# SoraKurihara/FFM

Hardware: AMD Instinct MI355X
Metric: agent-steps/sec (whole node), 12×12 grid × 64k envs, 1/2/4/8 GPU (higher is better)
Workload: dtype f32; 1 GPU; ffm_core step, 12x12 room, 32 agents/env, 65536 envs/GPU, neumann, Philox seed 42, on-device auto-reset, steady state (envs desynchronised by a 1000-step untimed burn-in after reset); burn_in_steps=1000, map=12x12, agents_per_env=32, envs_per_gpu=65536, global_envs=65536, parallelism=env-sharded x1

## Files before the change

ffm_amd/csrc/core_group.hip:

```cpp
#include <hip/hip_runtime.h>
#include <stdint.h>

#include <algorithm>
#include <cstdlib>
#include <cstring>

#include "core_common.h"
#include "kernels.h"
#include "lane_common.h"
#include "episode_log.h"
#include "wave_reset.h"

namespace ffm {

namespace {

constexpr int kGroupMaxIters = 16;
constexpr int kGroupPendWords = 8 * kGroupMaxIters / 32;

struct GroupCarve {
    size_t grid, tile, words, posst, kp, keys, pend, dummy, per_wave;
};

template <int G>
__host__ __device__ inline GroupCarve group_carve(int PHW, int TS, int F) {
    GroupCarve c;
    size_t o = 0;
    c.grid = o;  o += a16((size_t)G * PHW * 2);
    c.tile = o;  o += a16((size_t)G * TS * 4);
    c.keys = 0;
    const size_t keys_end = a16((size_t)(F > 0 ? F : 1) * 8);
    if (o < keys_end) o = keys_end;
    c.words = o; o += (size_t)G * 32 * 4;
    c.posst = o;
    c.kp = o;    o += a16((size_t)(((G * 32 + 63) / 64) * 64 + 1) * 2);
    c.pend = o;  o += kGroupPendWords * 4;
    c.dummy = o; o += 4;
    c.per_wave = a16(o);
    return c;
}

__host__ __device__ inline size_t group_shared_bytes(int PHW, int F) {
    return a16((size_t)PHW) + a16((size_t)PHW * 4) + a16((size_t)(F > 0 ? F : 1) * 2) + a16((size_t)PHW * 2);
}

constexpr int kGeomWords = 12;
constexpr int kGeomTableBytes = 64 * kGeomWords * 4;

template <int H, int W, int G>
void group_lane_geom(int lane, int32_t (&w)[kGeomWords]) {
    constexpr int HW = H * W, TS = lane_tile_floats(H, W), Q4 = HW / 4, Q = G * Q4;
    constexpr int NS = (Q + 63) / 64, NSF = Q / 64, HQ = (4 + W) / 4;
    static_assert(NS <= 3 && (4 + W) % 4 == 0 && TS % 4 == 0 && G * 2 * HQ <= 64 && G * TS / 4 <= 255,
                  "geometry table entry");
    uint32_t yfl = 0, senv = 0, tail = 0;
    int lo[3] = {0, 0, 0}, ro[3] = {0, 0, 0}, tlo = 0, tro = 0;
    for (int k = 0; k < 3; k++) w[k] = -1;
    for (int k = 0; k < NS; k++) {
        const int q = k * 64 + lane;
        const int s = q / Q4, c = 4 * (q - s * Q4), y = c % W;
        w[k] = q < Q ? s * TS + 4 + W + c : -1;
        yfl |= (q < Q && y == 0 ? 1u : 0u) << (2 * k);
        yfl |= (q < Q && y == W - 4 ? 2u : 0u) << (2 * k);
        senv |= (uint32_t)(q < Q ? s : 15) << (4 * k);
        lo[k] = q < Q && y != 0 ? w[k] - 1 : 0;
        ro[k] = q < Q && y != W - 4 ? w[k] + 4 : 0;
    }
    if (Q % 64 != 0 && (Q % 64) * 4 == 64) {
        const int q = 4 * 64 * NSF + lane;
        const int s = q / HW, c = q - s * HW, y = c % W, off = s * TS + 4 + W + c;
        tail = (y == 0 ? 1u : 0u) | (y == W - 1 ? 2u : 0u);
        tlo = y != 0 ? off - 1 : 0;
        tro = y != W - 1 ? off + 1 : 0;
    }
    const int s = lane / (2 * HQ), j = lane % (2 * HQ);
    const uint32_t halo = lane < G * 2 * HQ ? (uint32_t)(s * (TS / 4) + (j < HQ ? j : TS / 4 - 2 * HQ + j)) : 255u;
    w[3] = (int32_t)(yfl | (senv << 8) | (tail << 20) | (halo << 24));
    w[4] = lo[0]; w[5] = ro[0]; w[6] = lo[1]; w[7] = ro[1];
    w[8] = tlo; w[9] = tro; w[10] = lo[2]; w[11] = ro[2];
}

__device__ __forceinline__ int cs_pp(uint32_t v) { return (int)(v & 0xFFFFu); }
__device__ __forceinline__ int cs_al(uint32_t v) { return (int)((v >> 16) & 31u); }
__device__ __forceinline__ int cs_s(uint32_t v) { return (int)((v >> 21) & 7u); }
__device__ __forceinline__ bool cs_live(uint32_t v) { return ((v >> 24) & 1u) != 0u; }
__device__ __forceinline__ int cs_xp1(uint32_t v) { return (int)(v >> 25); }

}

#ifndef FFM_GROUP_PROBE_VALU
#define FFM_GROUP_PROBE_VALU 0
#endif
#ifndef FFM_GROUP_PROBE_SALU
#define FFM_GROUP_PROBE_SALU 0
#endif
#ifndef FFM_GROUP_PROBE_DUP
#define FFM_GROUP_PROBE_DUP 0
#endif

#ifndef FFM_GROUP_ABLATE
#define FFM_GROUP_ABLATE 0
#endif

#ifndef FFM_GROUP_TAIL
#define FFM_GROUP_TAIL 1
#endif

#ifndef FFM_GROUP_LADDER
#define FFM_GROUP_LADDER 4
#endif

#ifndef FFM_GROUP_PF
#define FFM_GROUP_PF 0
#endif

#ifndef FFM_GROUP_STAGGER
#define FFM_GROUP_STAGGER 0
#endif

#ifndef FFM_GROUP_WAVES
#define FFM_GROUP_WAVES 6
#endif

#ifndef FFM_GROUP_G
#define FFM_GROUP_G 4
#endif
constexpr int kGroupG = FFM_GROUP_G;
#ifndef FFM_GROUP_G_SMALL
#define FFM_GROUP_G_SMALL 2
#endif
constexpr int kGroupGSmall = FFM_GROUP_G_SMALL;

template <int NB, int HT, int WT, int G, bool KD1, bool EPL>
__global__ __launch_bounds__(256) __attribute__((amdgpu_waves_per_eu(FFM_GROUP_WAVES, 8)))
void core_group_kernel(CoreStepArgs a) {
    extern __shared__ __attribute__((aligned(16))) unsigned char smem[];
    constexpr int H = HT, W = WT, HW = H * W, PW = W + 2, PHW = (H + 2) * PW;
    constexpr int TS = lane_tile_floats(H, W);
    constexpr int Q4 = HW / 4;
    constexpr int Q = G * Q4;
    constexpr int NS = (Q + 63) / 64;
    constexpr int NSF = Q / 64;
    constexpr bool SCALAR_TAIL = NB == 4 && FFM_GROUP_TAIL && Q % 64 != 0 && (Q % 64) * 4 == 64;
    constexpr int MAXC = (G * 32 + 63) / 64;
    constexpr int PWORDS = G * 16;
    static_assert(G >= 1 && G <= 8 && HW % 4 == 0 && H + 1 < 128, "group geometry");
    static_assert(MAXC * 64 >= G * 32 && PWORDS * 4 <= (MAXC * 64 + 1) * 2, "kp spans the chunks; posst fits in it");
    const int A = a.A;
    const int lane = (int)(threadIdx.x & 63);
    const int wv = __builtin_amdgcn_readfirstlane((int)(threadIdx.x >> 6));

    const GroupCarve cv = group_carve<G>(PHW, TS, a.F);
    const float* psff = reinterpret_cast<const float*>(smem + a16((size_t)PHW));
    const uint16_t* pfree = reinterpret_cast<const uint16_t*>(smem + a16((size_t)PHW) + a16((size_t)PHW * 4));
    unsigned char* wbase = smem + group_shared_bytes(PHW, a.F) + (size_t)wv * cv.per_wave;
    uint16_t* const grid = reinterpret_cast<uint16_t*>(wbase + cv.grid);
    float* const tile = reinterpret_cast<float*>(wbase + cv.tile);
    uint32_t* const words = reinterpret_cast<uint32_t*>(wbase + cv.words);
    uint32_t* const posst32 = reinterpret_cast<uint32_t*>(wbase + cv.posst);
    const uint16_t* const posst = reinterpret_cast<const uint16_t*>(wbase + cv.posst);
    uint16_t* const kp = reinterpret_cast<uint16_t*>(wbase + cv.kp);
    unsigned long long* keys = reinterpret_cast<unsigned long long*>(wbase + cv.keys);
    uint32_t* const pend = reinterpret_cast<uint32_t*>(wbase + cv.pend);
    const int kDummy16 = (int)((cv.dummy - cv.grid) / 2);
    const int kDummy32 = (int)((cv.dummy - cv.words) / 4);

    static_assert(G == kGroupG || G == kGroupGSmall, "a geometry table per built group size");
    const int sq4 = a.stage_q4;
    const __amdgpu_buffer_rsrc_t rS = pair_rsrc(a.stage, sq4 * 16 + 2 * kGeomTableBytes);
    const int gtab = sq4 * 16 + (G == kGroupG ? kGeomTableBytes : 0);
    auto geom = [&](int j) {
        return __builtin_bit_cast(uint4, __builtin_amdgcn_raw_buffer_load_b128(rS, lane * 16 + j * 1024, gtab, 0));
    };
    const uint4 gw = geom(0);
    static_assert(NS <= 3, "geometry table entry");
    int toff[NS];
#pragma unroll
    for (int k = 0; k < NS; k++) toff[k] = (int)(k == 0 ? gw.x : k == 1 ? gw.y : gw.z);
    const uint32_t geo = gw.w;
    int lo[NS], ro[NS];
#pragma unroll
    for (int k = 0; k < NS; k++) lo[k] = ro[k] = 0;
    if (NB == 4) {
        const uint4 gb = geom(1);
        lo[0] = (int)gb.x; ro[0] = (int)gb.y;
        if (NS > 1) { lo[1] = (int)gb.z; ro[1] = (int)gb.w; }
        if (NS > 2 && !SCALAR_TAIL) {
            const uint4 gc = geom(2);
            lo[2] = (int)gc.z; ro[2] = (int)gc.w;
        }
    }

    const long long E = a.E;
    const uint32_t ebase = (uint32_t)a.env_base;
    const int Epad = (int)((E + 7) & ~7LL);
    const __amdgpu_buffer_rsrc_t rC = pair_rsrc(a.cnt, Epad * 4);
    const __amdgpu_buffer_rsrc_t rP = pair_rsrc(a.pos, Epad * A * 2 + 4);
    const __amdgpu_buffer_rsrc_t rD = pair_rsrc(a.dff, Epad * HW * 4);
    const int ngroups = (int)((E + G - 1) / G);
    const int wstride = (int)gridDim.x * 4;
    int g = (int)blockIdx.x * 4 + wv;

    struct GState {
        float4 d[NS];
        uint32_t p0, p1;
        int c;
    };
    const __amdgpu_buffer_rsrc_t rZ = pair_rsrc(a.dff, 0);
    auto load = [&](int gg, GState& st) {
        const bool ok = gg >= 0;
        const int e0 = ok ? gg * G : 0;
        const __amdgpu_buffer_rsrc_t rc = ok ? rC : rZ, rp = ok ? rP : rZ, rd = ok ? rD : rZ;
        st.c = (int)__builtin_amdgcn_raw_buffer_load_b32(rc, lane < G ? lane * 4 : kOOB, e0 * 4, 0);
        st.p0 = __builtin_amdgcn_raw_buffer_load_b32(rp, lane < PWORDS ? lane * 4 : kOOB, e0 * A * 2, 0);
        st.p1 = PWORDS > 64 ? __builtin_amdgcn_raw_buffer_load_b32(rp, 64 + lane < PWORDS ? 256 + lane * 4 : kOOB,
                                                                 e0 * A * 2, 0)
                            : 0u;
#pragma unroll
        for (int k = 0; k < NS; k++) {
            const int q = k * 64 + lane;
            st.d[k] = __builtin_bit_cast(float4,
                                         __builtin_amdgcn_raw_buffer_load_b128(rd, q < Q ? q * 16 : kOOB, e0 * HW * 4, 0));
        }
    };
    constexpr int LAD = FFM_GROUP_LADDER;
    constexpr int PF = FFM_GROUP_PF;
    if (FFM_GROUP_STAGGER > 0) {
        const int mine = g < ngroups ? (ngroups - 1 - g) / wstride + 1 : 0;
        const int most = (ngroups - 1) / wstride + 1;
        if (mine < most) __builtin_amdgcn_s_sleep(FFM_GROUP_STAGGER);
    }
    GState cur;
    load(g < ngroups ? g : -1, cur);

    if (LAD >= 1) {
    if ((int)threadIdx.x < sq4)
        reinterpret_cast<uint4*>(smem)[threadIdx.x] = __builtin_bit_cast(
            uint4, __builtin_amdgcn_raw_buffer_load_b128(rS, (int)threadIdx.x * 16, 0, 0));
    static_assert((PHW * 2) % 8 == 0 && PHW * 2 / 8 <= 64, "8-B grid copies, one per lane");
    if (lane < PHW * 2 / 8) {
        const int pm16 = (int)(a16((size_t)PHW) + a16((size_t)PHW * 4) + a16((size_t)(a.F > 0 ? a.F : 1) * 2));
        const auto mw = __builtin_amdgcn_raw_buffer_load_b64(rS, lane * 8, pm16, 0);
#pragma unroll
        for (int s = 0; s < G; s++)
            *reinterpret_cast<uint2*>(reinterpret_cast<unsigned char*>(grid) + s * (PHW * 2) + lane * 8) =
                __builtin_bit_cast(uint2, mw);
    }
    if ((geo >> 24) != 255u) reinterpret_cast<float4*>(tile)[geo >> 24] = make_float4(0.f, 0.f, 0.f, 0.f);
    if (lane < kGroupPendWords) pend[lane] = 0u;
    __syncthreads();
    }

    unsigned c_steps = 0, c_exits = 0, c_resets = 0;
    constexpr uint32_t mW = (uint32_t)(((1ull << 32) + (unsigned)W - 1) / (unsigned)W);
    const int g_first = g;
    for (int iter = 0; g < ngroups; g += wstride, iter++) {
        const int e0 = g * G;
        const int nenv = (int)min((long long)G, E - e0);
        if (LAD <= 2) {
            const __amdgpu_buffer_rsrc_t rq = pair_rsrc(a.pos + e0 * A, (nenv * A * 2 + 3) & ~3);
            __builtin_amdgcn_raw_buffer_store_b32(cur.p0, rq, lane < PWORDS ? lane * 4 : kOOB, 0, 0);
            if (PWORDS > 64)
                __builtin_amdgcn_raw_buffer_store_b32(cur.p1, rq, 64 + lane < PWORDS ? 256 + lane * 4 : kOOB, 0, 0);
            __builtin_amdgcn_raw_buffer_store_b32((unsigned)cur.c, pair_rsrc(a.cnt + e0, nenv * 4),
                                                  lane < G ? lane * 4 : kOOB, 0, 0);
            c_steps += (unsigned)A * (unsigned)nenv;
        }
        if (LAD <= 1) {
            const __amdgpu_buffer_rsrc_t rq = pair_rsrc(a.dff + e0 * HW, nenv * HW * 4);
#pragma unroll
            for (int k = 0; k < NS; k++) {
                const int q = k * 64 + lane;
                buf_st4(rq, q < Q ? q * 16 : kOOB, cur.d[k]);
            }
            GState nx;
            load(g + wstride < ngroups ? g + wstride : -1, nx);
            cur = nx;
            continue;
        }

        GState nxt;
        const int gn = g + wstride < ngroups ? g + wstride : -1;
#pragma unroll
        for (int k = 0; k < NS; k++)
            if (k < NSF || toff[k] >= 0) *reinterpret_cast<float4*>(tile + toff[k]) = cur.d[k];
        if (PF == 3) load(gn, nxt);
        unsigned long long rsm = 0ull;
        if (LAD == 2) wave_sync();
        if (LAD >= 3) {
        if (lane < PWORDS) posst32[lane] = cur.p0;
        if (PWORDS > 64 && 64 + lane < PWORDS) posst32[64 + lane] = cur.p1;
        int S[G + 1];
        S[0] = 0;
#pragma unroll
        for (int s = 0; s < G; s++) S[s + 1] = S[s] + __builtin_amdgcn_readlane(cur.c, s);
        const int T = S[G];
        c_steps += (unsigned)T;
        wave_sync();

        uint32_t cs[MAXC], cr[MAXC];
#pragma unroll
        for (int c = 0; c < MAXC; c++) {
            cs[c] = (uint32_t)(PW + 1) | (1u << 25);
            cr[c] = 15u;
            if (c * 64 < T) {
                const int j = c * 64 + lane;
                int s = 0, st = 0;
#pragma unroll
                for (int q = 1; q < G; q++) {
                    const bool ge = j >= S[q];
                    s += ge ? 1 : 0;
                    st = ge ? S[q] : st;
                }
                const bool live = j < T;
                const int al = live ? j - st : 0;
                const uint32_t p = posst[live ? s * A + al : 0];
                const int x = (int)__umulhi(p, mW);
                const int y = (int)p - x * W;
                const int pp = live ? (x + 1) * PW + y + 1 : PW + 1;
                grid[live ? s * PHW + pp : kDummy16] = (uint16_t)(DirCodes::kAgent | (uint32_t)al | (DirCodes::kNoDir << 8));
                cs[c] = (uint32_t)pp | ((uint32_t)al << 16) | ((uint32_t)s << 21) | ((live ? 1u : 0u) << 24) |
                        ((uint32_t)(live ? x + 1 : 1) << 25);
            }
        }
        wave_sync();

        if (PF == 2) load(gn, nxt);
#pragma unroll
        for (int c = 0; c < MAXC; c++) {
            if (LAD == 3) cr[c] = DirCodes::kNoDir;
            if (LAD >= 4 && c * 64 < T) {
                const uint32_t v = cs[c];
                const int pp = cs_pp(v), al = cs_al(v), s = cs_s(v);
                const bool live = cs_live(v);
                const uint32_t genv = ebase + (uint32_t)e0 + (uint32_t)s;
                const uint4 pb = philox(make_uint4(a.t, genv, (uint32_t)al, kPurDecide << 28), a.key0, a.key1);
                words[live ? s * 32 + al : kDummy32] = pb.w;
                const uint16_t* gk = grid + s * PHW;
                const float* dk = tile + s * TS;
                const int dd0 = 3 - 2 * cs_xp1(v);
                bool to_exit = false;
                uint32_t slot = lane_decide<NB, true, KD1>(pp, PW, gk, psff, dk, dd0, a.kS32, a.kD32, pb.x, to_exit);
                slot = live ? slot : kNoReq;
                if (slot == kPending)
                    slot = NB == 4 ? lane_decide_exact<NB, true>(pp, PW, gk, psff, dk, dd0, a.kS32, a.kD32,
                                                                 u53(pb.x, pb.y))
                                   : lane_decide_exact_arr<NB, true>(pp, PW, gk, psff, dk, dd0, a.kS32, a.kD32,
                                                               u53(pb.x, pb.y));
                const uint32_t sd = slot <= (uint32_t)NB ? slot : DirCodes::kNoDir;
                grid[live ? s * PHW + pp : kDummy16] =
                    (uint16_t)(DirCodes::kAgent | (uint32_t)al | (sd << 8) | ((pb.z >> 31) << 12));
                cr[c] = sd | ((to_exit ? 1u : 0u) << 4);
#if FFM_GROUP_PROBE_DUP
                if (c == MAXC - 1) {
                    uint32_t salt;
                    asm volatile("v_mov_b32 %0, 0" : "=v"(salt));
                    const uint4 pb2 = philox(make_uint4(a.t, genv, (uint32_t)al + salt, kPurDecide << 28), a.key0,
                                             a.key1);
                    bool te2 = false;
                    const uint32_t slot2 =
                        lane_decide<NB, true, KD1>(pp, PW, gk, psff, dk, dd0, a.kS32, a.kD32, pb2.x, te2);
                    asm volatile("" ::"v"(slot2), "v"(pb2.w), "v"(te2 ? 1u : 0u));
                }
#endif
            }
        }
        wave_sync();

        if (PF == 1) load(gn, nxt);
        unsigned long long km[MAXC];
        int kept = 0;
#pragma unroll
        for (int c = 0; c < MAXC; c++) {
            km[c] = 0ull;
            if (c * 64 < T) {
                const uint32_t v = cs[c];
                const int pp = cs_pp(v), al = cs_al(v), s = cs_s(v);
                const bool live = cs_live(v);
                const uint32_t sd = cr[c] & 15u;
                const bool to_exit = (cr[c] & 16u) != 0u;
                const uint32_t slot = sd == DirCodes::kNoDir ? (uint32_t)kNoReq : sd;
                const uint16_t* gk = grid + s * PHW;
                const int r = (int)slot_cell_k<NB, PW>(slot, pp);
                const bool req = slot <= (uint32_t)NB;
                const bool moving = req && r != pp;
                bool granted = req && !moving;
                if (LAD >= 4) {
                    const int rt = moving ? r : pp;
                    int m = 0, k = 0, o = 0x7F;
                    uint32_t zo = 0u;
#pragma unroll
                    for (int d = 0; d < NB; d++) {
                        const uint32_t cc = gk[rt - nb_dx<NB>(d) * PW - nb_dy<NB>(d)];
                        const bool is = (cc & DirCodes::kAgent) != 0u && ((cc >> 8) & 0xFu) == (uint32_t)d;
                        const int who = (int)(cc & DirCodes::kIdx);
                        m += is ? 1 : 0;
                        k += (is && who < al) ? 1 : 0;
                        const bool lower = is && who < o;
                        zo = lower ? (cc >> 12) & 1u : zo;
                        o = lower ? who : o;
                    }
                    granted = moving ? m == 1 : granted;
                    if (moving && m > 1) {
                        const uint32_t w = words[s * 32 + o];
                        const uint32_t genv = ebase + (uint32_t)e0 + (uint32_t)s;
                        const int kk = philox_friction(zo << 31, w, (uint32_t)m, a.key0, a.key1, a.t, genv,
                                                       (uint32_t)o);
                        granted = kk == k;
                    }
                }
                if (granted)
                    __hip_atomic_fetch_add(tile + s * TS + pp + 3 - 2 * cs_xp1(v), 1.0f, __ATOMIC_RELAXED,
                                           __HIP_MEMORY_SCOPE_WAVEFRONT);
                const int np = granted ? r : pp;
                const bool keep = live && !(granted && to_exit);
                km[c] = __ballot(keep);
                const int kpv = kept + lanes_below(km[c]);
                kept += __popcll(km[c]);
                cr[c] = (uint32_t)np | ((keep ? 1u : 0u) << 16) | ((uint32_t)kpv << 17);
            }
        }

#pragma unroll
        for (int c = 0; c < MAXC; c++) {
            if (c * 64 < T) {
                const uint32_t v = cs[c];
                kp[c * 64 + lane] = (uint16_t)(cr[c] >> 17);
                grid[cs_live(v) ? cs_s(v) * PHW + cs_pp(v) : kDummy16] = 0;
            }
        }
        if (lane == 0) kp[T] = (uint16_t)kept;
        c_exits += (unsigned)(T - kept);
        wave_sync();
#pragma unroll
        for (int c = 0; c < MAXC; c++) {
            if (c * 64 < T) {
                const uint32_t v = cs[c], w = cr[c];
                const int j = c * 64 + lane;
                const int s = cs_s(v);
                const bool keep = ((w >> 16) & 1u) != 0u;
                const int start = j - cs_al(v);
                const int newidx = (int)(w >> 17) - (int)kp[cs_live(v) ? start : 0];
                __builtin_amdgcn_raw_buffer_store_b16((uint16_t)unpad((int)(w & 0xFFFFu), PW), rP,
                                                      keep ? (s * A + newidx) * 2 : kOOB, e0 * A * 2, 0);
            }
        }
        int Sl = T, Sh = T;
#pragma unroll
        for (int s = 0; s < G; s++) {
            Sl = lane == s ? S[s] : Sl;
            Sh = lane == s ? S[s + 1] : Sh;
        }
        const int nk = (int)kp[Sh] - (int)kp[Sl];
        const bool rs = a.auto_reset && lane < nenv && nk == 0;
        rsm = __ballot(rs);
        __builtin_amdgcn_raw_buffer_store_b32((unsigned)(rs ? a.N : nk), rC, lane < G ? lane * 4 : kOOB, e0 * 4, 0);
        if (rsm) {
            c_resets += (unsigned)__popcll(rsm);
            if (a.episodes && rs) a.episodes[e0 + lane] += 1;
            if (lane == 0) pend[iter >> 2] |= (uint32_t)rsm << (8 * (iter & 3));
        }
        if (EPL && (rsm || !a.auto_reset))
            eplog_end_wave(a, lane < nenv && nk == 0 && Sh > Sl, rs, e0 + lane, a.t, lane);
        }

        if (PF == 0 || LAD < 3) load(gn, nxt);

#if FFM_GROUP_PROBE_VALU > 0 || FFM_GROUP_PROBE_SALU > 0
        {
            uint32_t pv = (uint32_t)lane, ps = (uint32_t)g;
#pragma unroll
            for (int i = 0; i < FFM_GROUP_PROBE_VALU; i++) asm volatile("v_add_u32 %0, %0, 1" : "+v"(pv));
#pragma unroll
            for (int i = 0; i < FFM_GROUP_PROBE_SALU; i++) asm volatile("s_add_u32 %0, %0, 1" : "+s"(ps));
            asm volatile("" ::"v"(pv), "s"(ps));
        }
#endif
        if (SCALAR_TAIL) {
            const int q = 4 * 64 * NSF + lane;
            constexpr int ts = 4 * 64 * NSF / HW, tc = 4 * 64 * NSF - ts * HW;
            static_assert(!SCALAR_TAIL || (4 * 64 * NSF + 63) / HW == ts, "the scalar tail spans envs");
            const float* p = tile + (ts * TS + 4 + W + tc) + lane;
            const float m0 = p[0], mu = p[-W], md = p[W], pl = p[-1], pr = p[1];
            const float ml = (geo & (1u << 20)) ? 0.0f : pl, mr = (geo & (2u << 20)) ? 0.0f : pr;
            const float b0 = a.c0 * m0, bu = a.c0 * mu, bd = a.c0 * md, bl = a.c0 * ml, br = a.c0 * mr;
            float acc = b0;
            acc = acc + a.c1 * bu;
            acc = acc + a.c1 * bd;
            acc = acc + a.c1 * bl;
            acc = acc + a.c1 * br;
            float o = acc < 1e-4f ? 0.0f : acc;
            if (rsm && ((rsm >> ts) & 1ull)) o = 0.0f;
            __builtin_amdgcn_raw_buffer_store_b32(__builtin_bit_cast(uint32_t, o), rD, q * 4, e0 * HW * 4, 0);
        }
#pragma unroll
        for (int k = 0; k < (SCALAR_TAIL ? NSF : NS); k++) {
            const int tb = toff[k];
            if (k >= NSF && tb < 0) continue;
            const bool yl = ((geo >> (2 * k)) & 1u) != 0u, yr = ((geo >> (2 * k)) & 2u) != 0u;
            const float* p = tile + tb;
            float b[3][6];
#pragma unroll
            for (int dx = -1; dx <= 1; dx++) {
                const float4 u = *reinterpret_cast<const float4*>(p + dx * W);
                b[dx + 1][1] = a.c0 * u.x; b[dx + 1][2] = a.c0 * u.y;
                b[dx + 1][3] = a.c0 * u.z; b[dx + 1][4] = a.c0 * u.w;
                if (NB == 4 && dx != 0) continue;
                b[dx + 1][0] = a.c0 * tile[NB == 4 ? lo[k] : yl ? 0 : tb + dx * W - 1];
                b[dx + 1][5] = a.c0 * tile[NB == 4 ? ro[k] : yr ? 0 : tb + dx * W + 4];
            }
            float o[4];
#pragma unroll
            for (int jj = 0; jj < 4; jj++) {
                float acc = b[1][jj + 1];
#pragma unroll
                for (int d = 0; d < NB; d++) {
                    const float t = a.c1 * b[1 + nb_dx<NB>(d)][jj + 1 + nb_dy<NB>(d)];
                    acc = acc + t;
                }
                o[jj] = acc < 1e-4f ? 0.0f : acc;
            }
            float4 out = make_float4(o[0], o[1], o[2], o[3]);
            if (rsm) {
                if ((rsm >> ((geo >> (8 + 4 * k)) & 15u)) & 1ull) out = make_float4(0.f, 0.f, 0.f, 0.f);
            }
            __builtin_amdgcn_raw_buffer_store_b128(__builtin_bit_cast(__attribute__((ext_vector_type(4))) unsigned, out),
                                                   rD, (k * 64 + lane) * 16, e0 * HW * 4, 0);
        }
        wave_sync();
        cur = nxt;
    }

    if (c_resets) wave_sync();
    for (int w = 0; w < (LAD >= 1 && c_resets ? kGroupPendWords : 0); w++) {
        uint32_t m = (uint32_t)__builtin_amdgcn_readfirstlane((int)pend[w]);
        while (m) {
            const int bit = w * 32 + __builtin_ctz(m);
            m &= m - 1u;
            const long long e = (long long)(g_first + (bit >> 3) * wstride) * G + (bit & 7);
            static_assert((H - 2) * (W - 2) <= 128, "wave_reset_env<.., SMALL>");
            wave_reset_env<PW, true>(a, ebase + (uint32_t)e, keys, pfree, a.pos + e * A, lane);
            if (FFM_GROUP_ABLATE & 1)
                wave_reset_env<PW, true>(a, ebase + (uint32_t)e, keys, pfree, a.pos + e * A, lane);
        }
    }

    if (lane == 0) {
        unsigned long long* ctr = a.counters + 4 * ((size_t)blockIdx.x * 4 + wv);
        if (c_steps) atomicAdd(&ctr[0], (unsigned long long)c_steps);
        if (c_exits) atomicAdd(&ctr[1], (unsigned long long)c_exits);
        if (c_resets) atomicAdd(&ctr[2], (unsigned long long)c_resets);
        if (blockIdx.x == 0 && wv == 0 && !a.no_step_count) atomicAdd(&ctr[3], 1ull);
    }
}

size_t core_group_smem_bytes(int H, int W, int F, int waves, int G) {
    const int PHW = (H + 2) * (W + 2);
    const size_t per_wave = G == kGroupGSmall ? group_carve<kGroupGSmall>(PHW, lane_tile_floats(H, W), F).per_wave
                                              : group_carve<kGroupG>(PHW, lane_tile_floats(H, W), F).per_wave;
    return group_shared_bytes(PHW, F) + (size_t)waves * per_wave;
}

bool core_group_supported(int H, int W) { return H == 12 && W == 12; }

int core_group_max_iters() { return kGroupMaxIters; }

int core_group_stage_q4(int H, int W, int F) { return (int)(group_shared_bytes((H + 2) * (W + 2), F) / 16); }

size_t core_group_stage_bytes(int H, int W, int F) {
    return group_shared_bytes((H + 2) * (W + 2), F) + 2 * (size_t)kGeomTableBytes;
}

void core_group_stage_build(int H, int W, int F, const uint8_t* pmap, const float* psff, float kS32,
                            const uint16_t* free_padded, unsigned char* out) {
    const int PHW = (H + 2) * (W + 2);
    std::memset(out, 0, core_group_stage_bytes(H, W, F));
    unsigned char* p = out;
    std::memcpy(p, pmap, (size_t)PHW);
    p += a16((size_t)PHW);
    for (int i = 0; i < PHW; i++) {
        const float v = kS32 * psff[i];
        std::memcpy(p + 4 * (size_t)i, &v, 4);
    }
    p += a16((size_t)PHW * 4);
    if (F > 0) std::memcpy(p, free_padded, (size_t)F * 2);
    p += a16((size_t)(F > 0 ? F : 1) * 2);
    for (int i = 0; i < PHW; i++) {
        const uint16_t v = pmap[i];
        std::memcpy(p + 2 * (size_t)i, &v, 2);
    }
    p += a16((size_t)PHW * 2);
    if (!core_group_supported(H, W)) return;
    for (int lane = 0; lane < 64; lane++) {
        int32_t w[kGeomWords];
        group_lane_geom<12, 12, kGroupGSmall>(lane, w);
        for (int j = 0; j < kGeomWords / 4; j++) std::memcpy(p + j * 1024 + lane * 16, w + 4 * j, 16);
        group_lane_geom<12, 12, kGroupG>(lane, w);
        for (int j = 0; j < kGeomWords / 4; j++) std::memcpy(p + kGeomTableBytes + j * 1024 + lane * 16, w + 4 * j, 16);
    }
}

template <int NB, bool KD1, int G>
static hipError_t group_op(const CoreStepArgs& a, int blocks, hipStream_t s, int op, int* occ) {
    const size_t smem = core_group_smem_bytes(a.H, a.W, a.F, 4, G);
    if (op) {
        *occ = 0;
        if (hipOccupancyMaxActiveBlocksPerMultiprocessor(occ, core_group_kernel<NB, 12, 12, G, KD1, false>, 256, smem) !=
            hipSuccess)
            *occ = 0;
        return hipSuccess;
    }
    const long long groups = (a.E + G - 1) / G;
    if (a.H != 12 || a.W != 12 || a.A > 32 || (groups + (long long)blocks * 4 - 1) / ((long long)blocks * 4) > kGroupMaxIters)
        return hipErrorInvalidConfiguration;
    if (!a.stage || a.stage_q4 != core_group_stage_q4(a.H, a.W, a.F) || a.stage_q4 > 256)
        return hipErrorInvalidConfiguration;
    if (a.ep_start) core_group_kernel<NB, 12, 12, G, KD1, true><<<dim3((unsigned)blocks), dim3(256), smem, s>>>(a);
    else core_group_kernel<NB, 12, 12, G, KD1, false><<<dim3((unsigned)blocks), dim3(256), smem, s>>>(a);
    return hipGetLastError();
}

template <int NB>
static hipError_t group_op_kd(const CoreStepArgs& a, int blocks, hipStream_t s, int op, int* occ, int G) {
    if (G == kGroupGSmall)
        return a.kD32 == 1.0f ? group_op<NB, true, kGroupGSmall>(a, blocks, s, op, occ)
                              : group_op<NB, false, kGroupGSmall>(a, blocks, s, op, occ);
    return a.kD32 == 1.0f ? group_op<NB, true, kGroupG>(a, blocks, s, op, occ)
                          : group_op<NB, false, kGroupG>(a, blocks, s, op, occ);
}

hipError_t launch_core_group(const CoreStepArgs& a, int nb, int blocks, hipStream_t s, int G) {
    return nb == 4 ? group_op_kd<4>(a, blocks, s, 0, nullptr, G) : group_op_kd<8>(a, blocks, s, 0, nullptr, G);
}

int core_group_blocks_per_cu(const CoreStepArgs& a, int nb, int G) {
    int n = 0;
    (void)(nb == 4 ? group_op_kd<4>(a, 0, nullptr, 1, &n, G) : group_op_kd<8>(a, 0, nullptr, 1, &n, G));
    return n;
}

int core_group_pick_envs(const CoreStepArgs& a, int nb, long long E, int cus) {
    if (const char* ov = std::getenv("FFM_GROUP_ENVS")) {
        const int v = std::atoi(ov);
        if (v == kGroupGSmall || v == kGroupG) return v;
    }
    const long long waves = (long long)cus * std::max(1, core_group_blocks_per_cu(a, nb, kGroupG)) * 4;
    return 2 * ((E + kGroupG - 1) / kGroupG) <= waves ? kGroupGSmall : kGroupG;
}

}
```

Baseline: 47.04 billion agent-steps/s.

## Resolve pending exact decisions cooperatively across wave lanes

When the fast lane_decide path leaves some lanes pending, the exact softmax/CDF fallback is no longer run divergently per lane. The wave now walks the pending lanes serially, and for each one spreads the five neighbour candidates across lanes 0-4, using readlane and ballot for the max, sum and CDF reductions. This avoids the divergent per-lane exact path, which serialises the whole wave. The cost is a serial loop over pending lanes, many readlane operations and a double-precision prefix that must match the per-lane exact result bit for bit. It is only active for NB==4.

```diff
diff --git a/ffm_amd/csrc/core_group.hip b/ffm_amd/csrc/core_group.hip
--- a/ffm_amd/csrc/core_group.hip
+++ b/ffm_amd/csrc/core_group.hip
@@ -86,6 +86,65 @@
 __device__ __forceinline__ bool cs_live(uint32_t v) { return ((v >> 24) & 1u) != 0u; }
 __device__ __forceinline__ int cs_xp1(uint32_t v) { return (int)(v >> 25); }
 
+__device__ __forceinline__ float lane_f32(float x, int l) {
+    return __builtin_bit_cast(float, __builtin_amdgcn_readlane(__builtin_bit_cast(int, x), l));
+}
+
+template <int W, int PHW, int TS>
+__device__ __forceinline__ uint32_t group_exact_coop(unsigned long long pend, uint32_t slot, uint32_t csv, uint32_t wx,
+                                                     uint32_t wy, const uint16_t* grid, const float* psff,
+                                                     const float* tile, float kD, int lane) {
+    constexpr int NB = 4, PW = W + 2;
+    while (pend) {
+        const int L = __builtin_ctzll(pend);
+        pend &= pend - 1ull;
+        int ln = lane;
+        asm volatile("" : "+v"(ln));
+        const int off = ln == 0 ? -PW : ln == 1 ? PW : ln == 2 ? -1 : ln == 3 ? 1 : 0;
+        const int doff = ln == 0 ? -W : ln == 1 ? W : ln == 2 ? -1 : ln == 3 ? 1 : 0;
+        const uint32_t v = (uint32_t)__builtin_amdgcn_readlane((int)csv, L);
+        const int pp = cs_pp(v), s = cs_s(v), dd0 = 3 - 2 * cs_xp1(v);
+        const int cell = pp + off;
+        const uint32_t g = grid[s * PHW + cell];
+        const unsigned vm = ((unsigned)__ballot(g == 0u || g == 3u) & ((1u << NB) - 1u)) | (1u << NB);
+        const float sa = psff[cell];
+        const float sb = kD * tile[s * TS + pp + dd0 + doff];
+        const float sc = sa + sb;
+        float mx = -__builtin_inff();
+#pragma unroll
+        for (int k = 0; k <= NB; k++) {
+            const float sk = lane_f32(sc, k);
+            mx = (((vm >> k) & 1u) && sk > mx) ? sk : mx;
+        }
+        const float e = np_expf(sc - mx);
+        float sum = -0.0f;
+#pragma unroll
+        for (int k = 0; k <= NB; k++) {
+            const float t = sum + lane_f32(e, k);
+            sum = ((vm >> k) & 1u) ? t : sum;
+        }
+        const float p = e / sum;
+        const unsigned vmk = vm & ((2u << (ln & 7)) - 1u);
+        double run = 0.0;
+#pragma unroll
+        for (int k = 0; k <= NB; k++) {
+            const double t = run + (double)lane_f32(p, k);
+            run = ((vmk >> k) & 1u) ? t : run;
+        }
+        const unsigned long long rb = __builtin_bit_cast(unsigned long long, run);
+        const double last = __builtin_bit_cast(
+            double, ((unsigned long long)(uint32_t)__builtin_amdgcn_readlane((int)(uint32_t)(rb >> 32), NB) << 32) |
+                        (uint32_t)__builtin_amdgcn_readlane((int)(uint32_t)rb, NB));
+        const double inv = 1.0 / last;
+        const double u = u53((uint32_t)__builtin_amdgcn_readlane((int)wx, L),
+                             (uint32_t)__builtin_amdgcn_readlane((int)wy, L));
+        const unsigned gt = (unsigned)__ballot(cdf_gt(run, last, inv, u)) & vm & ((1u << NB) - 1u);
+        const uint32_t pick = gt ? (uint32_t)__builtin_ctz(gt) : (uint32_t)NB;
+        slot = lane == L ? pick : slot;
+    }
+    return slot;
+}
+
 }
 
 #ifndef FFM_GROUP_PROBE_VALU
@@ -120,6 +179,10 @@
 
 #ifndef FFM_GROUP_WAVES
 #define FFM_GROUP_WAVES 6
+#endif
+
+#ifndef FFM_GROUP_COOP_EXACT
+#define FFM_GROUP_COOP_EXACT 1
 #endif
 
 #ifndef FFM_GROUP_G
@@ -342,7 +405,11 @@
                 bool to_exit = false;
                 uint32_t slot = lane_decide<NB, true, KD1>(pp, PW, gk, psff, dk, dd0, a.kS32, a.kD32, pb.x, to_exit);
                 slot = live ? slot : kNoReq;
-                if (slot == kPending)
+                if (NB == 4 && FFM_GROUP_COOP_EXACT) {
+                    const unsigned long long pm = __ballot(slot == kPending);
+                    if (pm)
+                        slot = group_exact_coop<W, PHW, TS>(pm, slot, v, pb.x, pb.y, grid, psff, tile, a.kD32, lane);
+                } else if (slot == kPending)
                     slot = NB == 4 ? lane_decide_exact<NB, true>(pp, PW, gk, psff, dk, dd0, a.kS32, a.kD32,
                                                                  u53(pb.x, pb.y))
                                    : lane_decide_exact_arr<NB, true>(pp, PW, gk, psff, dk, dd0, a.kS32, a.kD32,
```

New measurement: 52.22 billion agent-steps/s, median of 6. 1.11x the previous value.
